# HowToSD/cremage

Hardware: AMD Instinct MI355X
Metric: images/sec SD1.5 512x512 20-step Euler ancestral (txt2img, CFG 7.5, incl. VAE decode) (higher is better)
Workload: dtype bf16; 1 GPU; SD1.5 txt2img 512x512, batch 4 per GPU, 20-step Euler ancestral, bf16 UNet (B=8 with CFG) + fp32-class (split-bf16 x3) VAE decode, synthetic name-keyed weights, synthetic conditioning; sampler=euler_a, sampler_steps=20, parallelism=batch-sharded x1 (weights broadcast 0.00 GB once, images all-gathered per step)

## Files before the change

### cremage_amd/_lib.py

```python
import ctypes as C
import os

_HERE = os.path.dirname(os.path.abspath(__file__))
HALF_F16 = os.environ.get("CRG_HALF", "bf16").lower() in ("f16", "fp16", "float16", "half")
LIB_PATH = os.path.abspath(os.environ["CRG_LIB"]) if os.environ.get("CRG_LIB") else os.path.join(_HERE, "libcrg_hip_f16.so" if HALF_F16 else "libcrg_hip.so")

BF16, F32, F16 = 0, 1, 2
PREC_BF16, PREC_BF16X3, PREC_F16MX = 0, 1, 2
EPI_NONE, EPI_SILU, EPI_GEGLU = 0, 1, 2
BIAS_NONE, BIAS_COL, BIAS_ROW = 0, 1, 2
PACK_LINEAR, PACK_CONV, PACK_GEGLU = 0, 1, 2
K_SLOTS = 17
SLOT_NAMES = ["gemm_w1", "gemm_w4", "gemm_w5", "gemm_x3", "conv_w1", "conv_w4", "conv_w5", "conv_x3", "splitk_reduce", "attention",
              "gn_stats", "gn_apply", "layernorm", "elementwise", "conv_small", "softmax", "lngemm"]
SLOT_FAMILY = ["gemm", "gemm", "gemm", "gemm", "conv", "conv", "conv", "conv", "splitk_reduce", "attention", "groupnorm", "groupnorm",
               "layernorm", "elementwise", "conv_small", "softmax", "gemm"]

c_void_p, c_int, c_int64, c_float, c_size_t = C.c_void_p, C.c_int, C.c_int64, C.c_float, C.c_size_t


class GemmArgs(C.Structure):
    _fields_ = [
        ("a", c_void_p), ("lda", c_int64), ("a_bstride", c_int64),
        ("w", c_void_p), ("ldw", c_int64), ("w_bstride", c_int64),
# ... 80 lines not shown
                              c_int, c_float, c_int, c_int]),
    "crg_groupnorm_split": (c_int, [c_void_p, c_void_p, c_void_p, c_void_p, c_int, c_void_p, c_void_p, c_void_p, c_void_p, c_int, c_int, c_int,
                                    c_int, c_float, c_int]),
    "crg_groupnorm_pre_split": (c_int, [c_void_p, c_void_p, c_void_p, c_void_p, c_void_p, c_void_p, c_void_p, c_void_p, c_int, c_int, c_int, c_int,
                                        c_float, c_int]),
    "crg_groupnorm_pre": (c_int, [c_void_p, c_void_p, c_void_p, c_void_p, c_int, c_void_p, c_void_p, c_void_p, c_void_p, c_void_p, c_int, c_int,
                                  c_int, c_int, c_float, c_int, c_int, c_int, c_int]),
    "crg_split_bf16": (c_int, [c_void_p, c_void_p, c_void_p, c_void_p, c_void_p, c_int64]),
    "crg_split_mx": (c_int, [c_void_p, c_void_p, c_void_p, c_void_p, c_void_p, c_int64, c_int, c_int, c_int]),
    "crg_groupnorm_mx": (c_int, [c_void_p, c_void_p, c_void_p, c_void_p, c_void_p, c_void_p, c_void_p, c_void_p, c_int, c_int, c_int, c_int, c_float,
                                 c_int, c_int, c_int]),
    "crg_pack_weight_mx": (c_int, [c_void_p, c_void_p, c_void_p, c_int, c_int, c_int, c_void_p, c_void_p, c_int, c_int]),
    "crg_layernorm": (c_int, [c_void_p, c_void_p, c_void_p, c_void_p, c_void_p, c_void_p, c_int64, c_int, c_float, c_int]),
    "crg_gemm": (c_int, [c_void_p, c_void_p, C.POINTER(GemmArgs)]),
    "crg_conv2d": (c_int, [c_void_p, c_void_p, C.POINTER(ConvArgs)]),
    "crg_ln_gemm": (c_int, [c_void_p, c_void_p, C.POINTER(LnGemmArgs)]),
    "crg_pack_weight": (c_int, [c_void_p, c_void_p, c_void_p, c_int, c_int, c_int, c_int, c_int, c_void_p, c_void_p]),
    "crg_pack_geglu_bias": (c_int, [c_void_p, c_void_p, c_void_p, c_int, c_void_p]),
    "crg_pack_ln_weight": (c_int, [c_void_p, c_void_p, c_void_p, c_int, c_void_p, c_void_p, c_void_p, c_int, c_int, c_int, c_void_p, c_void_p, c_void_p]),
    "crg_attention": (c_int, [c_void_p, c_void_p, c_void_p, c_int64, c_void_p, c_int64, c_void_p, c_int64, c_void_p, c_int64,
                              c_int, c_int, c_int, c_int, c_int, c_float, c_int]),
    "crg_attention_v": (c_int, [c_void_p, c_void_p, c_void_p, c_int64, c_void_p, c_int64, c_void_p, c_int64, c_void_p, c_int64,
                              c_int, c_int, c_int, c_int, c_int, c_float, c_int]),
    "crg_softmax_rows": (c_int, [c_void_p, c_void_p, c_void_p, c_void_p, c_int64, c_int, c_int64, c_float, c_int]),
    "crg_conv_small": (c_int, [c_void_p, c_void_p, c_void_p, c_void_p, c_void_p, c_void_p, c_int, c_int, c_int, c_int, c_int,
                               c_int, c_int, c_int]),
    "crg_timestep_embedding": (c_int, [c_void_p, c_void_p, c_void_p, c_void_p, c_int, c_int, c_int]),
    "crg_silu": (c_int, [c_void_p, c_void_p, c_void_p, c_void_p, c_int64, c_int]),
    "crg_nchw_to_nhwc": (c_int, [c_void_p, c_void_p, c_void_p, c_void_p, c_int, c_int, c_int, c_int, c_int]),
    "crg_nhwc_to_nchw": (c_int, [c_void_p, c_void_p, c_void_p, c_void_p, c_int, c_int, c_int, c_int, c_int]),
# ... 70 lines not shown
```

### cremage_amd/csrc/crg_api.hip

```cpp
#include "crg_common.h"

int crg_fail(crg_ctx* ctx, int code, const char* fmt, ...) {
  if (ctx) {
    char buf[1024];
    va_list ap;
    va_start(ap, fmt);
    vsnprintf(buf, sizeof(buf), fmt, ap);
    va_end(ap);
    ctx->err = buf;
  }
  return code;
}

void* crg_scratch(crg_ctx* ctx, size_t bytes) {
  if (ctx->scratch_bytes >= bytes) return ctx->scratch;
  size_t want = ctx->scratch_bytes ? ctx->scratch_bytes * 2 : (size_t(64) << 20);
  while (want < bytes) want *= 2;
  void* fresh = nullptr;
  if (hipMalloc(&fresh, want) != hipSuccess) return nullptr;
  if (ctx->scratch) ctx->retired.push_back(ctx->scratch);
  ctx->scratch = fresh;
  ctx->scratch_bytes = want;
  return ctx->scratch;
}
// ... 187 lines not shown
template <typename ST>
__global__ __launch_bounds__(256) void pack_mx_kernel(const ST* __restrict__ src, _Float16* __restrict__ w16, unsigned char* __restrict__ w8,
                                                      int n_in, long total8, float sh, float sl) {
  const int kk = 9 * n_in;
  for (long i = (long)blockIdx.x * 256 + threadIdx.x; i < total8; i += (long)gridDim.x * 256) {
    const long d = i * 8;
    const int o = (int)(d / kk), k = (int)(d - (long)o * kk);
    const int chunk = k / (9 * 64), r = k - chunk * 9 * 64, tap = r / 64, c0 = r - tap * 64;
    float f[8];
#pragma unroll
    for (int e = 0; e < 8; ++e) f[e] = (float)src[((long)o * n_in + chunk * 64 + c0 + e) * 9 + tap];
    crg_store_mx8(f, w16 + d, w8 + 2 * (d - c0) + c0, sh, sl);
  }
}

}

extern "C" int crg_pack_weight_mx(crg_ctx* ctx, void* stream, const void* src, int src_dtype, int n_out, int n_in, void* dst16, void* dst8,
                                  int hi_log2, int lo_log2) {
  if (!ctx) return -22;
  CRG_REQUIRE(ctx, src && dst16 && dst8 && n_out > 0 && n_in > 0 && n_in % 64 == 0, "pack_weight_mx: 3x3 conv weights with Cin %% 64 == 0 (got %d)", n_in);
  const long total8 = (long)n_out * n_in * 9 / 8;
  const int grid = (int)((total8 + 255) / 256 < 4096 ? (total8 + 255) / 256 : 4096);
  hipStream_t st = (hipStream_t)stream;
  const float sh = ldexpf(1.f, hi_log2), sl = ldexpf(1.f, lo_log2);
  if (src_dtype == CRG_F32) hipLaunchKernelGGL(pack_mx_kernel<float>, dim3(grid), dim3(256), 0, st, (const float*)src, (_Float16*)dst16, (unsigned char*)dst8, n_in, total8, sh, sl);
  else if (src_dtype == CRG_BF16) hipLaunchKernelGGL(pack_mx_kernel<bf16>, dim3(grid), dim3(256), 0, st, (const bf16*)src, (_Float16*)dst16, (unsigned char*)dst8, n_in, total8, sh, sl);
  else if (src_dtype == CRG_F16) hipLaunchKernelGGL(pack_mx_kernel<_Float16>, dim3(grid), dim3(256), 0, st, (const _Float16*)src, (_Float16*)dst16, (unsigned char*)dst8, n_in, total8, sh, sl);
  else return crg_fail(ctx, -22, "pack_weight_mx: unsupported source dtype %d", src_dtype);
  CRG_CHECK_LAUNCH(ctx, "pack_weight_mx");
// ... 53 lines not shown
```

### cremage_amd/csrc/gemm_conv.hip

```cpp
#include "gemm_shared.h"
#include <cstdlib>

namespace {
using namespace crg_mm;



__device__ __forceinline__ bf16x8 split_hi(const crg_vec8<float>& v, bf16x8& lo) {
  bf16x8 hi;
#pragma unroll
  for (int i = 0; i < 8; ++i) {
    float f = v.get(i);
    bf16 h = (bf16)f;
    hi[i] = h;
    lo[i] = (bf16)(f - (float)h);
  }
  return hi;
}


template <int WNT, int NSPLIT, typename AT, typename YT, bool CONV, int KG>
__global__ __launch_bounds__(256 * KG) void gemm_kernel(GemmP p) {
  constexpr int BN = 32 * WNT;
  constexpr int RS = 32 * KG;
// ... 622 lines not shown
              V[(long)(n + e) * p.vt_ld] = (bf16)v;
            }
          }
        }
      }
      return;
    }
  }
  if constexpr (PAIR) {
    gemm_epilogue_pairs<WNT, WMT, GST ? 1 : 0, RST>(p, acc, m0, n0, wm, wn, frow, fq, bz, r2, r1, pre_res, bpre, pre_bias);
  } else {
    gemm_epilogue<WNT, YT, WMT>(p, acc, m0, n0, wm, wn, frow, fq, bz, sid, rres, pre_res, bpre, pre_bias);
  }
}

template <int WNT, typename YT, bool PAIR, int NS = 1, int KG = 1, int MT = 1, bool MX = false>
__global__ __launch_bounds__(256 * KG * MT, (KG == 1 && MT == 1) ? 2 : 1) void conv3_rowhalo_kernel(GemmP p) {
  static_assert(!PAIR || (sizeof(YT) == 2 && NS == 1), "paired columns: bf16 output, single-plane operands");
  static_assert(MT == 1 || (KG == 1 && NS == 1), "256-row tiles: single-plane operands, no in-block split-K");
  static_assert(!MX || (NS == 2 && KG == 2 && MT == 1), "MX: the split-plane form on two k-groups");
  constexpr int WMT = 4, NW = 4 * KG * MT;
  constexpr int TP = 128 * MT;
  constexpr int BN = 32 * WNT;
  constexpr int WS_BYTES = BN * 128;
  constexpr int WRG = BN / 8;
  constexpr int WL = (WRG + NW - 1) / NW;
  constexpr int XI = ((MT == 2 ? 36 : 20) + NW - 1) / NW;
  extern __shared__ __attribute__((aligned(16))) char smem[];
  typedef const __attribute__((address_space(1))) void* gptr_t;
  typedef __attribute__((address_space(3))) void* lptr_t;

  const int t = threadIdx.x;
  const int lane = t & 63;
  const int wave = __builtin_amdgcn_readfirstlane(t >> 6);
  const int kg = MT == 2 ? 0 : wave >> 2;
  const int wm = MT == 2 ? wave >> 1 : (wave & 3) >> 1, wn = wave & 1;
  const int Wd = p.Wo, Hd = p.Ho, sh = p.up ? 1 : 0;
  const bool lin = p.halo_lin != 0;
  const bool seg = lin || Wd > TP;
  const int WP = seg ? TP + 2 : Wd + 2;
  const int R = seg ? 1 : TP / Wd;
  const int xpix = R * WP;
  const int XP = (xpix + 7) >> 3;
  const int xbuf_bytes = XP * 1024;
  char* const wring = smem;
  char* const xbuf = smem + 2 * NS * WS_BYTES;

  int tile_m, tile_n, sid;
  block_to_tile(p, tile_m, tile_n, sid);
  const int m0 = tile_m * TP, n0 = tile_n * BN;
  const int bz = 0;
  const bf16* Wp = p.w;
  const long a_lo_off = NS == 2 ? reinterpret_cast<const bf16*>(p.a_lo) - reinterpret_cast<const bf16*>(p.a) : 0;
  const long w_lo_off = NS == 2 ? p.w_lo - p.w : 0;
  const bf16* zpage = p.zero_page;
  const int rsub = lane >> 3;
  const int clog = (lane & 7) ^ rsub;

  int xsrc[XI];
  int xh[XI];
  unsigned xmask[XI];
  {
    const int rows_total = p.M / Wd;
    const int row0 = m0 / Wd;
    const int w0 = m0 - row0 * Wd;
#pragma unroll
    for (int i = 0; i < XI; ++i) {
// ... 20 lines not shown
    }
  }
  bool wok[WL];
  long wrow_off[WL];
#pragma unroll
  for (int q = 0; q < WL; ++q) {
    const int pos = (wave + NW * q) * 8 + rsub;
    const int n = n0 + (PAIR ? unpair_col<WNT>(pos) : pos);
    wok[q] = n < p.N && (wave + NW * q) < WRG;
    wrow_off[q] = (long)n * p.ldw;
  }
  const int g_begin = sid * p.ks_q + (sid < p.ks_r ? sid : p.ks_r);
  const int g_end = g_begin + p.ks_q + (sid < p.ks_r ? 1 : 0);

  auto stage_x = [&](int g, int slot) {
    const int c = g / 3, kh = g - 3 * c;
    const int cch = c * 64 + clog * 8;
    const bool second = cch >= p.C1;
    const bf16* base = reinterpret_cast<const bf16*>(second ? p.x2 : p.a);
    const int Cs = second ? p.C2 : p.C1;
    const int cs = second ? cch - p.C1 : cch;
    char* xb = xbuf + ((g - g_begin) & 1) * (NS * xbuf_bytes);
#pragma unroll
    for (int i = 0; i < XI; ++i) {
      if (i % 3 != slot) continue;
      const int jp = wave + NW * i;
      if (jp < XP) {
        const bool ok = (xmask[i] >> kh) & 1u;
        const bf16* src = ok ? base + (long)(xsrc[i] + ((xh[i] + kh - 1) >> sh) * p.W) * Cs + cs : zpage;
        __builtin_amdgcn_global_load_lds((gptr_t)src, (lptr_t)(xb + jp * 1024), 16, 0, 0);
        if constexpr (NS == 2) {
          const bf16* src2 = ok ? src + a_lo_off : zpage;
          __builtin_amdgcn_global_load_lds((gptr_t)src2, (lptr_t)(xb + xbuf_bytes + jp * 1024), 16, 0, 0);
        }
      }
    }
  };
  auto stage_w = [&](int kt, int buf) {
    char* ws = wring + buf * (NS * WS_BYTES);
    const long kc = (long)kt * BK + clog * 8;
// ... 11 lines not shown
  };

  f32x4 acc[WNT][WMT];
#pragma unroll
  for (int i = 0; i < WNT; ++i)
#pragma unroll
    for (int j = 0; j < WMT; ++j) acc[i][j] = f32x4{0.f, 0.f, 0.f, 0.f};

  const int frow = lane & 15;
  const int fq = lane >> 4;
  int xb0[WMT];
#pragma unroll
  for (int j = 0; j < WMT; ++j) {
    const int ml = wm * 64 + j * 16 + frow;
    const int r = seg ? 0 : ml / Wd;
    xb0[j] = r * WP + (ml - r * Wd);
  }
  unsigned edge = 0;
  if (lin) {
#pragma unroll
    for (int j = 0; j < WMT; ++j) {
      const int m = m0 + wm * 64 + j * 16 + frow;
      const int wcol = m % Wd;
      edge |= (wcol == 0 ? 1u : 0u) << j;
      edge |= (wcol == Wd - 1 ? 1u : 0u) << (8 + j);
    }
  }

  bf16x4 rres[PAIR ? 1 : WNT][PAIR ? 1 : WMT];
  bf16x8 r2[PAIR ? (WNT / 2 > 0 ? WNT / 2 : 1) : 1][PAIR ? WMT : 1];
  bf16x4 r1[PAIR ? WMT : 1];
// ... 25 lines not shown
            rres[i][j] = *reinterpret_cast<const bf16x4*>(Rm + (n + 4 <= p.N ? n : p.N - 4));
          }
        }
      }
    }
    if (pre_bias) {
#pragma unroll
      for (int i = 0; i < WNT; ++i) {
        const int n = (PAIR && i < 2 * (WNT / 2)) ? nb + 32 * (i >> 1) + 8 * fq + 4 * (i & 1) : nb + 16 * i + 4 * fq;
        bpre[i] = *reinterpret_cast<const f32x4*>(p.bias + (n + 4 <= p.N ? n : p.N - 4));
      }
    }
  }

  if (g_begin < g_end) {
    stage_x(g_begin, 0);
    stage_x(g_begin, 1);
    stage_x(g_begin, 2);
    stage_w(3 * g_begin, 0);
  }
#ifdef CRG_X3_NOSTAGGER
  constexpr bool STAG = false;
#else
  constexpr bool STAG = KG == 2 && WNT == 4 && !MX;
#endif
  constexpr bool LO = NS == 2 && !MX;
  bf16x8 sxf[STAG ? WMT : 1], swf[STAG ? WNT : 1], sxl[STAG && LO ? WMT : 1], swl[STAG && LO ? WNT : 1];
  if constexpr (STAG) {
#pragma unroll
    for (int j = 0; j < WMT; ++j) { sxf[j] = bf16x8{0, 0, 0, 0, 0, 0, 0, 0}; if constexpr (LO) sxl[j] = sxf[j]; }
#pragma unroll
    for (int i = 0; i < WNT; ++i) { swf[i] = bf16x8{0, 0, 0, 0, 0, 0, 0, 0}; if constexpr (LO) swl[i] = swf[i]; }
  }
  typedef int v8i __attribute__((ext_vector_type(8)));
// ... 56 lines not shown
            acc[i][j] = CRG_MFMA_16x16x32(swl[i], sxf[j], acc[i][j]);
            acc[i][j] = CRG_MFMA_16x16x32(swf[i], sxl[j], acc[i][j]);
          }
          if constexpr (MX) acc[i][j] = __builtin_amdgcn_mfma_f32_16x16x32_f16(__builtin_bit_cast(h16x8, swf[i]), __builtin_bit_cast(h16x8, sxf[j]), acc[i][j], 0, 0, 0);
          else acc[i][j] = CRG_MFMA_16x16x32(swf[i], sxf[j], acc[i][j]);
        }
      mx_cross();
    }
  };
  int wbuf = 0;
  auto k_loop = [&](auto GBc) {
  constexpr bool GB = decltype(GBc)::value;
  for (int g = g_begin; g < g_end; ++g) {
    const char* xs = xbuf + ((g - g_begin) & 1) * (NS * xbuf_bytes);
#pragma unroll
    for (int kw = 0; kw < 3; ++kw) {
      wait_vmcnt<0>();
      asm volatile("" ::: "memory");
      __builtin_amdgcn_s_barrier();
      asm volatile("" ::: "memory");
      __builtin_amdgcn_s_setprio(2);
      if (kw < 2 || g + 1 < g_end) stage_w(3 * g + kw + 1, wbuf ^ 1);
      if (g + 1 < g_end) stage_x(g + 1, kw);
      __builtin_amdgcn_s_setprio(0);
      const char* ws = wring + wbuf * (NS * WS_BYTES);
      if constexpr (STAG) {
        auto stag_reads = [&]() {
#pragma unroll
          for (int j = 0; j < WMT; ++j) {
            const int off = lds_off(xb0[j] + kw, kg * 4 + fq);
            sxf[j] = *reinterpret_cast<const bf16x8*>(xs + off);
            if constexpr (LO) sxl[j] = *reinterpret_cast<const bf16x8*>(xs + xbuf_bytes + off);
          }
          if (kw != 1 && lin) {
#pragma unroll
            for (int j = 0; j < WMT; ++j) {
              if ((edge >> (kw == 0 ? j : 8 + j)) & 1u) {
// ... 84 lines not shown
#pragma unroll
      for (int i = 0; i < WNT; ++i)
#pragma unroll
        for (int j = 0; j < WMT; ++j) red[(i * WMT + j) * 64] = acc[i][j];
    }
    __syncthreads();
    if (kg == 1) return;
#pragma unroll
    for (int i = 0; i < WNT; ++i)
#pragma unroll
      for (int j = 0; j < WMT; ++j) acc[i][j] += red[(i * WMT + j) * 64];
  }
  if constexpr (PAIR) {
    gemm_epilogue_pairs<WNT, WMT>(p, acc, m0, n0, wm, wn, frow, fq, bz, r2, r1, pre_res, bpre, pre_bias);
  } else {
    gemm_epilogue<WNT, YT, WMT>(p, acc, m0, n0, wm, wn, frow, fq, bz, sid, rres, pre_res, bpre, pre_bias);
  }
}

template <typename YT>
__global__ __launch_bounds__(256) void splitk_reduce_kernel(GemmP p) {
  const int n4 = p.N >> 2;
  const long srows = p.M - p.slab_row0;
  const long total = srows * n4;
  const int bz = blockIdx.y;
  const float* S = p.slab + (long)bz * p.splits * srows * p.N - (long)p.slab_row0 * p.N;
  YT* Y = reinterpret_cast<YT*>(p.y) + (long)bz * p.y_bs;
  const YT* R = p.res ? reinterpret_cast<const YT*>(p.res) + (long)bz * p.r_bs : nullptr;
  for (long idx = (long)blockIdx.x * 256 + threadIdx.x; idx < total; idx += (long)gridDim.x * 256) {
    const int mr = (int)(idx / n4);
    const int m = mr + p.slab_row0;
// ... 552 lines not shown
    p.pair = 0;
    crg_prof_scope ps(ctx, st, CONV ? CRG_K_CONV_X3 : CRG_K_GEMM_X3, wk.flops, wk.bytes);
    hipLaunchKernelGGL(kern, dim3(p.tiles_n * p.tiles_m * p.splits, batch, 1), dim3(512), lds_bytes, st, p);
    CRG_CHECK_LAUNCH(ctx, "gemm(planes)");
  }
  if (p.splits > 1) {
    const long total4 = (long)p.M * (p.N >> 2);
    const int rg = (int)((total4 + 255) / 256 > 2048 ? 2048 : (total4 + 255) / 256);
    crg_prof_scope ps(ctx, st, CRG_K_SPLITK, (double)batch * p.splits * p.M * p.N, (double)batch * p.M * p.N * (4.0 * p.splits + 4));
    hipLaunchKernelGGL(splitk_reduce_kernel<float>, dim3(rg, batch), dim3(256), 0, st, p);
    CRG_CHECK_LAUNCH(ctx, "splitk_reduce");
  }
  return 0;
}

template <int NSPLIT, typename AT, typename YT, bool CONV>
int launch_wnt(crg_ctx* ctx, hipStream_t st, GemmP& p, int batch, Work wk) {
  const bool geglu = p.epi == CRG_EPI_GEGLU;
  if (!geglu && p.N <= 32) return launch<1, NSPLIT, AT, YT, CONV>(ctx, st, p, batch, wk);
  if (!geglu && p.N % 160 == 0) return launch<5, NSPLIT, AT, YT, CONV>(ctx, st, p, batch, wk);
  return launch<4, NSPLIT, AT, YT, CONV>(ctx, st, p, batch, wk);
}

template <bool CONV>
int dispatch(crg_ctx* ctx, hipStream_t st, GemmP& p, int batch, int a_dtype, int y_dtype, int prec, Work wk) {
  const bool gstat_bf16 = prec == CRG_PREC_BF16 && a_dtype == CRG_BF16 && y_dtype == CRG_BF16 && (p.N & 7) == 0;
  const bool gstat_planes = (prec == CRG_PREC_BF16X3 || prec == CRG_PREC_F16MX) && a_dtype == CRG_BF16 && y_dtype == CRG_F32 && p.a_lo && !p.a_is_weight && (p.N & 3) == 0;
  if (p.gstat && !((gstat_bf16 || gstat_planes) && batch == 1 && p.epi == CRG_EPI_NONE))
    return crg_fail(ctx, -22, "gemm/conv: GroupNorm statistics need bf16 in / out (N %% 8 == 0) or pre-split planes in / fp32 out (N %% 4 == 0), batch 1 and a plain epilogue");
  if (prec == CRG_PREC_BF16) {
// ... 142 lines not shown
    CRG_REQUIRE(ctx, (((uintptr_t)a->gn_gamma | (uintptr_t)a->gn_beta | (uintptr_t)a->gn_y) & 15) == 0, "conv2d: GroupNorm pointers must be 16-byte aligned");
    p.gn_gamma = a->gn_gamma; p.gn_beta = a->gn_beta; p.gn_eps = a->gn_eps; p.gn_groups = a->gn_groups; p.gn_silu = a->gn_silu;
    p.gn_hw = a->Ho * a->Wo; p.gn_y = a->gn_y;
  }
  const double flops = 2.0 * p.M * (double)p.N * p.K;
  const double bytes = (double)a->N * a->H * a->W * Ctot * crg_dtype_size(a->x_dtype) + (double)p.N * p.K * 2 +
                       (double)p.M * p.N * crg_dtype_size(a->y_dtype) * (a->residual ? 2 : 1);
  ctx->gn_fused = false;
  const int rc = dispatch<true>(ctx, (hipStream_t)stream, p, 1, a->x_dtype, a->y_dtype, a->prec,
                                Work{flops, bytes, (double)a->N * a->H * a->W * Ctot * crg_dtype_size(a->x_dtype), (double)p.N * p.K * 2});
  if (a->gn_stats_rows) *a->gn_stats_rows = p.gstat_rows;
  if (rc || !a->gn_y || ctx->gn_fused) return rc;
  return crg_groupnorm(ctx, stream, a->y, nullptr, a->Cout, a->gn_gamma, a->gn_beta, a->gn_y, a->N, a->Ho * a->Wo, a->Cout, a->gn_groups,
                       a->gn_eps, a->gn_silu, a->y_dtype);
}
```

### cremage_amd/csrc/gemm_shared.h

```cpp
#pragma once
#include "crg_common.h"
#include <type_traits>

namespace crg_mm {

struct GemmP {
  const void* a; const void* a_lo; long lda, a_bs;
  const bf16* w; const bf16* w_lo; long ldw, w_bs;
  const float* bias; int bias_mode;
  const void* res; long ldr, r_bs;
  void* y; long ldy, y_bs;
  int M, N, K, epi;
  const float* cvec; int cvec_rows; long cvec_ld;
  const bf16* zero_page;
  int splits; float* slab;
  int a_is_weight;
  const void* x2; int C1, C2, Ctot, H, W, Ho, Wo, ks, stride, pad_t, pad_l, up;
  int cm;
  int tiles_n, tiles_m;
  int tile_base, tile_count, slab_row0;
  int pair;
  int rowhalo;
  int halo_lin;
  int ks_q, ks_r;
// ... 37 lines not shown
  }
}

__device__ __forceinline__ int lds_off(int row, int chunk) { return row * 128 + ((chunk ^ (row & 7)) << 4); }

__device__ __forceinline__ float row16_sum(float v) {
#if defined(__HIP_DEVICE_COMPILE__)
  v += __builtin_bit_cast(float, __builtin_amdgcn_update_dpp(0, __builtin_bit_cast(int, v), 0xB1, 0xF, 0xF, true));
  v += __builtin_bit_cast(float, __builtin_amdgcn_update_dpp(0, __builtin_bit_cast(int, v), 0x4E, 0xF, 0xF, true));
  v += __builtin_bit_cast(float, __builtin_amdgcn_update_dpp(0, __builtin_bit_cast(int, v), 0x141, 0xF, 0xF, true));
  v += __builtin_bit_cast(float, __builtin_amdgcn_update_dpp(0, __builtin_bit_cast(int, v), 0x140, 0xF, 0xF, true));
#endif
  return v;
}

template <int WNT, typename YT, int WMT = 4>
__device__ __forceinline__ void gemm_epilogue(const GemmP& p, f32x4 (&acc)[WNT][WMT], int m0, int n0, int wm, int wn, int frow, int fq,
                                              int bz, int sid, const bf16x4 (&pre)[WNT][WMT], bool use_pre,
                                              const f32x4 (&bpre)[WNT], bool use_bpre) {
  if (p.splits > 1) {
    const long srows = p.M - p.slab_row0;
    float* S = p.slab + ((long)bz * p.splits + sid) * srows * p.N - (long)p.slab_row0 * p.N;
#pragma unroll
    for (int j = 0; j < WMT; ++j) {
      const int m = m0 + wm * (16 * WMT) + j * 16 + frow;
      if (m >= p.M) continue;
#pragma unroll
      for (int i = 0; i < WNT; ++i) {
        const int n = n0 + wn * (16 * WNT) + i * 16 + fq * 4;
        if (n + 4 <= p.N) {
          *reinterpret_cast<f32x4*>(S + (long)m * p.N + n) = acc[i][j];
        } else {
          for (int e = 0; e < 4 && n + e < p.N; ++e) S[(long)m * p.N + n + e] = acc[i][j][e];
        }
      }
    }
    return;
  }
  YT* Y = reinterpret_cast<YT*>(p.y) + (long)bz * p.y_bs;
  const YT* R = p.res ? reinterpret_cast<const YT*>(p.res) + (long)bz * p.r_bs : nullptr;
  constexpr bool CAN_STATS = sizeof(YT) == 4 && (WMT % 2 == 0);
  const bool do_stats = CAN_STATS && p.gstat != nullptr;
  f32x4 gs1[CAN_STATS ? WNT : 1], gs2[CAN_STATS ? WNT : 1];
  auto flush_stats = [&](int jb) {
    if constexpr (CAN_STATS) {
      const int row0 = m0 + wm * (16 * WMT) + jb * 16;
      const long rb = row0 >> 5;
#pragma unroll
      for (int i = 0; i < WNT; ++i) {
        f32x4 a, b;
#pragma unroll
        for (int e = 0; e < 4; ++e) {
          a[e] = row16_sum(gs1[i][e]);
          b[e] = row16_sum(gs2[i][e]);
        }
        const int n = n0 + wn * (16 * WNT) + i * 16 + fq * 4;
        if (frow == 0 && n + 4 <= p.N && row0 < p.M) {
          *reinterpret_cast<f32x4*>(p.gstat + rb * p.N + n) = a;
          *reinterpret_cast<f32x4*>(p.gstat + p.gstat_plane + rb * p.N + n) = b;
        }
      }
    }
  };
#pragma unroll
  for (int j = 0; j < WMT; ++j) {
    const int m = m0 + wm * (16 * WMT) + j * 16 + frow;
    if constexpr (CAN_STATS) {
      if (do_stats && (j & 1) == 0) {
        if (j > 0) flush_stats(j - 2);
#pragma unroll
        for (int i = 0; i < WNT; ++i) gs1[i] = gs2[i] = f32x4{0.f, 0.f, 0.f, 0.f};
      }
    }
    if (m >= p.M) continue;
    const float brow = (p.bias_mode == CRG_BIAS_ROW) ? p.bias[m] : 0.f;
    const float* cv = p.cvec ? p.cvec + (long)(m / p.cvec_rows) * p.cvec_ld : nullptr;
    if (p.epi == CRG_EPI_GEGLU) {
      if constexpr (WNT % 2 == 0) {
#pragma unroll
        for (int u = 0; u < WNT / 2; ++u) {
          const int pn = n0 + wn * (16 * WNT) + u * 32 + fq * 4;
          if (pn >= p.N) continue;
          const int jn = (n0 + wn * (16 * WNT)) / 2 + u * 16 + fq * 4;
          f32x4 v = acc[2 * u][j], g = acc[2 * u + 1][j];
          if (p.bias_mode == CRG_BIAS_COL) {
            v += *reinterpret_cast<const f32x4*>(p.bias + pn);
            g += *reinterpret_cast<const f32x4*>(p.bias + pn + 16);
          }
          YT out[4];
// ... 9 lines not shown
#pragma unroll
    for (int i = 0; i < WNT; ++i) {
      const int n = n0 + wn * (16 * WNT) + i * 16 + fq * 4;
      if (n >= p.N) continue;
      f32x4 v = acc[i][j];
      const bool full = (n + 4 <= p.N);
      if (full) {
        if (use_bpre) v += bpre[i];
        else if (p.bias_mode == CRG_BIAS_COL) v += *reinterpret_cast<const f32x4*>(p.bias + n);
        else if (p.bias_mode == CRG_BIAS_ROW) v += brow;
        if (p.epi == CRG_EPI_SILU) {
#pragma unroll
          for (int e = 0; e < 4; ++e) v[e] = crg_silu_f(v[e]);
        }
        if (cv) v += *reinterpret_cast<const f32x4*>(cv + n);
        const long yo = (long)m * p.ldy + n;
        if (use_pre) {
#pragma unroll
          for (int e = 0; e < 4; ++e) v[e] += (float)pre[i][j][e];
        } else if (R) {
          const YT* rp = R + (long)m * p.ldr + n;
          if (((p.ldr | n) & 3) == 0) {
            if constexpr (sizeof(YT) == 2) {
              bf16x4 r4 = *reinterpret_cast<const bf16x4*>(rp);
#pragma unroll
              for (int e = 0; e < 4; ++e) v[e] += (float)r4[e];
            } else {
              v += *reinterpret_cast<const f32x4*>(rp);
            }
          } else {
#pragma unroll
// ... 15 lines not shown
          } else {
            *reinterpret_cast<f32x4*>(Y + yo) = v;
          }
        } else {
#pragma unroll
          for (int e = 0; e < 4; ++e) Y[yo + e] = (YT)v[e];
        }
      } else {
        for (int e = 0; e < 4 && n + e < p.N; ++e) {
          float s = v[e];
          if (p.bias_mode == CRG_BIAS_COL) s += p.bias[n + e];
          else if (p.bias_mode == CRG_BIAS_ROW) s += brow;
          if (p.epi == CRG_EPI_SILU) s = crg_silu_f(s);
          if (cv) s += cv[n + e];
          if (R) s += (float)R[(long)m * p.ldr + n + e];
          Y[(long)m * p.ldy + n + e] = (YT)s;
        }
      }
    }
  }
  if constexpr (CAN_STATS) {
    if (do_stats) flush_stats(WMT - 2);
  }
}

template <int WNT>
__device__ __forceinline__ int unpair_col(int pos) {
  const int w = pos / (16 * WNT);
  const int l = pos - w * (16 * WNT);
  if (l >= 32 * (WNT / 2)) return pos;
  const int g = l >> 5, t = (l >> 4) & 1, rho = l & 15;
// ... 239 lines not shown
```

### cremage_amd/ops.py

```python
from __future__ import annotations

import ctypes as C
from typing import Optional, Tuple

import torch

from . import _lib as L

HALF = torch.float16 if L.HALF_F16 else torch.bfloat16
_DT = {HALF: L.BF16, torch.float32: L.F32}
if not L.HALF_F16:
    _DT[torch.float16] = L.F16


def _dt(t: torch.Tensor) -> int:
    try:
        return _DT[t.dtype]
    except KeyError:
        raise L.CrgError(f"unsupported dtype {t.dtype}")


def _act_dt(t: torch.Tensor) -> int:
    if t.dtype not in (HALF, torch.float32):
        raise L.CrgError(f"activations must be {HALF} or float32, got {t.dtype}")
# ... 191 lines not shown
    src = w.detach().contiguous()
    if src.dtype not in _DT:
        src = src.float()
    n_out = src.shape[0]
    if kind == L.PACK_CONV:
        n_in, ks = src.shape[1], src.shape[2]
        cols = n_in * ks * ks
    else:
        n_in, ks = src[0].numel(), 1
        cols = n_in
    hi = torch.empty((n_out, cols), dtype=HALF, device=w.device)
    lo = torch.empty_like(hi) if split else None
    h = _h(w)
    L.check(L.load().crg_pack_weight(h, _st(), _p(src), _dt(src), kind, n_out, n_in, ks, _p(hi), _p(lo)), h, "crg_pack_weight")
    return _pack_cache.put((w,), (kind, split), (hi, lo))


VAE_MX = __import__("os").environ.get("CRG_VAE_MX", "0") != "0"
MX_X_LOG2 = (4, 15)


def packed_weight_mx(w: torch.Tensor):
    _need_cuda(w)
    r = _pack_cache.get((w,), ("mx",))
    if r is not None:
        return r
    src = w.detach().contiguous()
    if src.dtype not in _DT:
        src = src.float()
    n_out, n_in = src.shape[0], src.shape[1]
# ... 437 lines not shown
    ho = (hv + pt + pb - ks) // stride + 1
    wo = (wv + pl + pr - ks) // stride + 1
    if cin <= 8 or (cin == 9 and cout % 8 == 0) or (cout <= 8 and (cin % 8 != 0 or cin < 64)):
        if x_lo is not None:
            raise L.CrgError("conv2d: thin-channel convs take the fp32 tensor, not split planes")
        if stride != 1 or upsample2x or x2 is not None or cvec is not None or residual is not None or gn is not None or (pt, pl, pb, pr) != (ks // 2,) * 4:
            raise L.CrgError("conv2d: thin-channel convs support only stride 1, 'same' padding, no fusions (no fused GroupNorm either)")
        y = empty_image(n, cout, ho, wo, x.dtype, x.device)
        w32 = f32_vec(weight)
        h = _h(x)
        L.check(L.load().crg_conv_small(h, _st(), _p(x), _p(w32), _p(f32_vec(bias)), _p(y), n, hh, ww, cin, cout, ks, _act_dt(x),
                                        _act_dt(y)), h, "crg_conv_small")
        return y
    planes = x_lo is not None
    split = planes or x.dtype == torch.float32
    hi, lo = packed_weight(weight, L.PACK_CONV, split)
    y = empty_image(n, cout, ho, wo, torch.float32 if planes else x.dtype, x.device)
    if residual is not None:
        residual = to_channels_last(residual)
        if residual.shape != y.shape or residual.dtype != y.dtype:
            raise L.CrgError("conv2d: residual must match the output in shape and dtype")
    if cvec is not None:
        if cvec.dtype != torch.float32 or tuple(cvec.shape) != (n, cout) or cvec.stride(1) != 1 or cvec.stride(0) % 4:
            raise L.CrgError("conv2d: cvec must be fp32 [N, Cout] with unit column stride and 16-byte aligned rows")
    a = L.ConvArgs(x=x.data_ptr(), x2=x2.data_ptr() if x2 is not None else None, C1=c1, C2=c2, w=hi.data_ptr(),
                   w_lo=lo.data_ptr() if lo is not None else None, bias=_p(f32_vec(bias)).value, cvec=_p(cvec).value,
                   cvec_ld=cvec.stride(0) if cvec is not None else 0, residual=_p(residual).value, y=y.data_ptr(), N=n, H=hh, W=ww, Cout=cout, Ho=ho, Wo=wo, ksize=ks, stride=stride,
                   pad_t=pt, pad_l=pl, upsample2x=int(upsample2x), x_dtype=_act_dt(x), y_dtype=_act_dt(y),
                   prec=L.PREC_BF16X3 if planes else _prec(x), x_lo=x_lo.data_ptr() if planes else None)
    y_norm = keep = None
    if gn is not None:
# ... 1 lines not shown
        if planes or y.dtype != HALF or cout % groups or (cout // groups) % 8:
            raise L.CrgError("conv2d: the fused GroupNorm takes bf16 outputs with 8-aligned groups")
        y_norm = empty_image(n, cout, ho, wo, y.dtype, x.device)
        keep = (f32_vec(gw), f32_vec(gb))
        a.gn_gamma, a.gn_beta, a.gn_y = keep[0].data_ptr(), keep[1].data_ptr(), y_norm.data_ptr()
        a.gn_groups, a.gn_silu, a.gn_eps = int(groups), int(bool(silu)), float(eps)
    stats = _gn_stats_buffer(n * ho * wo, cout, ho * wo, x.dtype, y.dtype, x.device) if (gn_stats and gn is None and (planes or x.dtype == HALF)) else None
    if stats is not None and planes and (cout % 4 or VAE_GN_STATS is False):
        stats = None
    rows = C.c_int(32)
    if stats is not None:
        a.gn_stats = stats.data_ptr()
        if GN_TILE and not planes:
            a.gn_stats_rows = C.pointer(rows)
    h = _h(x)
    L.check(L.load().crg_conv2d(h, _st(), C.byref(a)), h, "crg_conv2d")
    if stats is not None:
        y._crg_gn = (stats, y._version, ho * wo, rows.value)
    return y if gn is None else (y, y_norm)


def _conv2d_mx(x16, x8, weight, bias, stride, padding, upsample2x, x2, cvec, residual, x_lo, gn_stats, gn):
    x16 = to_channels_last(x16)
    n, c, hh, ww = x16.shape
    cout, cin, ks, _ = weight.shape
    if x16.dtype != torch.float16 or x8.dtype != torch.uint8 or tuple(x8.shape) != (n, hh, ww, 2 * c) or not x8.is_contiguous():
        raise L.CrgError("conv2d(x_mx=): x must be the fp16 plane [N, C, H, W] (channels-last) and x_mx the uint8 plane [N, H, W, 2 C]")
    if ks != 3 or stride != 1 or padding not in (1, (1, 1, 1, 1)) or upsample2x or x2 is not None or x_lo is not None or gn is not None or cvec is not None \
            or cin != c or c % 64:
        raise L.CrgError("conv2d(x_mx=): 3x3 / stride 1 / pad 1 convs with Cin % 64 == 0 only (no upsample / concat / fused GroupNorm)")
    w16, w8, whi, wlo = packed_weight_mx(weight)
# ... 251 lines not shown
```

### include/crg_hip.h

```cpp
#ifndef CRG_HIP_H
#define CRG_HIP_H

#include <stddef.h>
#include <stdint.h>

#ifdef __cplusplus
extern "C" {
#endif

#define CRG_VERSION 103

typedef struct crg_ctx crg_ctx;

enum crg_dtype { CRG_BF16 = 0, CRG_F32 = 1, CRG_F16 = 2 };

enum crg_prec { CRG_PREC_BF16 = 0, CRG_PREC_BF16X3 = 1,
                CRG_PREC_F16MX = 2 };

enum crg_epilogue {
  CRG_EPI_NONE = 0,
  CRG_EPI_SILU = 1,
  CRG_EPI_GEGLU = 2
};

// ... 86 lines not shown
  int64_t cvec_ld;
  const void* residual;
  void* y;
  int N, H, W, Cout, Ho, Wo;
  int ksize, stride, pad_t, pad_l;
  int upsample2x;
  int x_dtype, y_dtype, prec;
  const void* x_lo;
  float* gn_stats;
  const float* gn_gamma; const float* gn_beta; void* gn_y;
  int gn_groups; int gn_silu; float gn_eps;
  int mx_log2[4];
  int* gn_stats_rows;
} crg_conv_args;
int crg_conv2d(crg_ctx* ctx, void* stream, const crg_conv_args* args);

enum crg_pack_kind { CRG_PACK_LINEAR = 0, CRG_PACK_CONV = 1, CRG_PACK_GEGLU = 2 };
int crg_pack_weight(crg_ctx* ctx, void* stream, const void* src, int src_dtype, int kind, int n_out, int n_in,
                    int ksize, void* dst_hi, void* dst_lo);
int crg_pack_geglu_bias(crg_ctx* ctx, void* stream, const float* src, int n_out2, float* dst);
int crg_pack_ln_weight(crg_ctx* ctx, void* stream, const void* src, int src_dtype, const float* gamma, const float* beta,
                       const float* bias, int kind, int n_out, int n_in, void* dst_w, float* dst_colsum, float* dst_bias);

int crg_attention(crg_ctx* ctx, void* stream, const void* q, int64_t ldq, const void* k, int64_t ldk,
                  const void* vt, int64_t ldvt, void* o, int64_t ldo, int B, int H, int Nq, int Nk, int Dh,
                  float scale, int dtype);
int crg_attention_v(crg_ctx* ctx, void* stream, const void* q, int64_t ldq, const void* k, int64_t ldk,
                    const void* v, int64_t ldv, void* o, int64_t ldo, int B, int H, int Nq, int Nk, int Dh,
                    float scale, int dtype);

int crg_softmax_rows(crg_ctx* ctx, void* stream, const void* x, void* y, int64_t rows, int cols, int64_t ld,
                     float scale, int dtype);

int crg_conv_small(crg_ctx* ctx, void* stream, const void* x, const float* w, const float* bias, void* y,
// ... 52 lines not shown
```

Baseline: 17.87 images/s.

## Fold nearest-2x upsample into VAE 3x3 conv via sub-pixel 2x2 weight classes

Replaces the nearest-upsample-then-3x3-conv in the VAE decoder with four 2x2 convolutions on the low-resolution input, one per output sub-pixel phase. The weights are pre-summed per phase into a packed hi/lo bf16 layout, and the epilogue scatters rows to interleaved output positions and to matching GroupNorm stat blocks. This cuts conv K from 9*Cin to 4*Cin per output pixel and avoids reading an upsampled image. The cost is a new kernel specialisation and a pre-summed weight pack whose rounding differs slightly from the plain path.

```diff
diff --git a/cremage_amd/_lib.py b/cremage_amd/_lib.py
--- a/cremage_amd/_lib.py
+++ b/cremage_amd/_lib.py
@@ -118,6 +118,8 @@
     "crg_layernorm": (c_int, [c_void_p, c_void_p, c_void_p, c_void_p, c_void_p, c_void_p, c_int64, c_int, c_float, c_int]),
     "crg_gemm": (c_int, [c_void_p, c_void_p, C.POINTER(GemmArgs)]),
     "crg_conv2d": (c_int, [c_void_p, c_void_p, C.POINTER(ConvArgs)]),
+    "crg_conv2d_subpix": (c_int, [c_void_p, c_void_p, C.POINTER(ConvArgs)]),
+    "crg_pack_weight_subpix": (c_int, [c_void_p, c_void_p, c_void_p, c_int, c_int, c_int, c_void_p, c_void_p]),
     "crg_ln_gemm": (c_int, [c_void_p, c_void_p, C.POINTER(LnGemmArgs)]),
     "crg_pack_weight": (c_int, [c_void_p, c_void_p, c_void_p, c_int, c_int, c_int, c_int, c_int, c_void_p, c_void_p]),
     "crg_pack_geglu_bias": (c_int, [c_void_p, c_void_p, c_void_p, c_int, c_void_p]),
diff --git a/cremage_amd/csrc/crg_api.hip b/cremage_amd/csrc/crg_api.hip
--- a/cremage_amd/csrc/crg_api.hip
+++ b/cremage_amd/csrc/crg_api.hip
@@ -225,6 +225,42 @@
   }
 }
 
+template <typename ST>
+__global__ __launch_bounds__(256) void pack_subpix_kernel(const ST* __restrict__ src, bf16* __restrict__ hi, bf16* __restrict__ lo, int n_out,
+                                                          int n_in, long total) {
+  for (long d = (long)blockIdx.x * 256 + threadIdx.x; d < total; d += (long)gridDim.x * 256) {
+    const long kk = 4L * n_in;
+    const long co = d / kk;
+    const int k = (int)(d - co * kk);
+    const int cls = (int)(co / n_out), o = (int)(co - (long)cls * n_out);
+    const int chunk = k >> 8, tap = (k >> 6) & 3, ci = chunk * 64 + (k & 63);
+    const int a = cls >> 1, b = cls & 1, r = tap >> 1, t = tap & 1;
+    const int h0 = a == 0 ? (r == 0 ? 0 : 1) : (r == 0 ? 0 : 2), h1 = a == 0 ? (r == 0 ? 0 : 2) : (r == 0 ? 1 : 2);
+    const int w0 = b == 0 ? (t == 0 ? 0 : 1) : (t == 0 ? 0 : 2), w1 = b == 0 ? (t == 0 ? 0 : 2) : (t == 0 ? 1 : 2);
+    const ST* s = src + ((long)o * n_in + ci) * 9;
+    float f = 0.f;
+    for (int kh = h0; kh <= h1; ++kh)
+      for (int kw = w0; kw <= w1; ++kw) f += (float)s[kh * 3 + kw];
+    const bf16 h = (bf16)f;
+    hi[d] = h;
+    lo[d] = (bf16)(f - (float)h);
+  }
+}
+
+}
+
+extern "C" int crg_pack_weight_subpix(crg_ctx* ctx, void* stream, const void* src, int src_dtype, int n_out, int n_in, void* dst_hi, void* dst_lo) {
+  if (!ctx) return -22;
+  CRG_REQUIRE(ctx, src && dst_hi && dst_lo && n_out > 0 && n_in > 0 && n_in % 64 == 0, "pack_weight_subpix: 3x3 conv weights with Cin %% 64 == 0 (got %d)", n_in);
+  const long total = 16L * n_out * n_in;
+  const int grid = (int)((total + 255) / 256 < 4096 ? (total + 255) / 256 : 4096);
+  hipStream_t st = (hipStream_t)stream;
+  if (src_dtype == CRG_F32) hipLaunchKernelGGL(pack_subpix_kernel<float>, dim3(grid), dim3(256), 0, st, (const float*)src, (bf16*)dst_hi, (bf16*)dst_lo, n_out, n_in, total);
+  else if (src_dtype == CRG_BF16) hipLaunchKernelGGL(pack_subpix_kernel<bf16>, dim3(grid), dim3(256), 0, st, (const bf16*)src, (bf16*)dst_hi, (bf16*)dst_lo, n_out, n_in, total);
+  else if (src_dtype == CRG_F16) hipLaunchKernelGGL(pack_subpix_kernel<_Float16>, dim3(grid), dim3(256), 0, st, (const _Float16*)src, (bf16*)dst_hi, (bf16*)dst_lo, n_out, n_in, total);
+  else return crg_fail(ctx, -22, "pack_weight_subpix: unsupported source dtype %d", src_dtype);
+  CRG_CHECK_LAUNCH(ctx, "pack_weight_subpix");
+  return 0;
 }
 
 extern "C" int crg_pack_weight_mx(crg_ctx* ctx, void* stream, const void* src, int src_dtype, int n_out, int n_in, void* dst16, void* dst8,
diff --git a/cremage_amd/csrc/gemm_conv.hip b/cremage_amd/csrc/gemm_conv.hip
--- a/cremage_amd/csrc/gemm_conv.hip
+++ b/cremage_amd/csrc/gemm_conv.hip
@@ -660,11 +660,13 @@
   }
 }
 
-template <int WNT, typename YT, bool PAIR, int NS = 1, int KG = 1, int MT = 1, bool MX = false>
+template <int WNT, typename YT, bool PAIR, int NS = 1, int KG = 1, int MT = 1, bool MX = false, bool SUB = false>
 __global__ __launch_bounds__(256 * KG * MT, (KG == 1 && MT == 1) ? 2 : 1) void conv3_rowhalo_kernel(GemmP p) {
   static_assert(!PAIR || (sizeof(YT) == 2 && NS == 1), "paired columns: bf16 output, single-plane operands");
   static_assert(MT == 1 || (KG == 1 && NS == 1), "256-row tiles: single-plane operands, no in-block split-K");
   static_assert(!MX || (NS == 2 && KG == 2 && MT == 1), "MX: the split-plane form on two k-groups");
+  static_assert(!SUB || (NS == 2 && KG == 2 && MT == 1 && !MX && !PAIR), "sub-pixel upsample: the bf16 x 3 split-plane form");
+  constexpr int KW = SUB ? 2 : 3;
   constexpr int WMT = 4, NW = 4 * KG * MT;
   constexpr int TP = 128 * MT;
   constexpr int BN = 32 * WNT;
@@ -681,8 +683,8 @@
   const int wave = __builtin_amdgcn_readfirstlane(t >> 6);
   const int kg = MT == 2 ? 0 : wave >> 2;
   const int wm = MT == 2 ? wave >> 1 : (wave & 3) >> 1, wn = wave & 1;
-  const int Wd = p.Wo, Hd = p.Ho, sh = p.up ? 1 : 0;
-  const bool lin = p.halo_lin != 0;
+  const int Wd = SUB ? p.W : p.Wo, Hd = SUB ? p.H : p.Ho, sh = (p.up && !SUB) ? 1 : 0;
+  const bool lin = !SUB && p.halo_lin != 0;
   const bool seg = lin || Wd > TP;
   const int WP = seg ? TP + 2 : Wd + 2;
   const int R = seg ? 1 : TP / Wd;
@@ -694,9 +696,15 @@
 
   int tile_m, tile_n, sid;
   block_to_tile(p, tile_m, tile_n, sid);
+  int cls = 0;
+  if constexpr (SUB) {
+    cls = tile_m & 3;
+    tile_m >>= 2;
+  }
+  const int pa = cls >> 1, pb = cls & 1;
   const int m0 = tile_m * TP, n0 = tile_n * BN;
   const int bz = 0;
-  const bf16* Wp = p.w;
+  const bf16* Wp = p.w + (SUB ? (long)cls * p.N * p.ldw : 0);
   const long a_lo_off = NS == 2 ? reinterpret_cast<const bf16*>(p.a_lo) - reinterpret_cast<const bf16*>(p.a) : 0;
   const long w_lo_off = NS == 2 ? p.w_lo - p.w : 0;
   const bf16* zpage = p.zero_page;
@@ -747,7 +755,7 @@
   const int g_end = g_begin + p.ks_q + (sid < p.ks_r ? 1 : 0);
 
   auto stage_x = [&](int g, int slot) {
-    const int c = g / 3, kh = g - 3 * c;
+    const int c = g / KW, kh = (g - KW * c) + (SUB ? pa : 0);
     const int cch = c * 64 + clog * 8;
     const bool second = cch >= p.C1;
     const bf16* base = reinterpret_cast<const bf16*>(second ? p.x2 : p.a);
@@ -756,7 +764,7 @@
     char* xb = xbuf + ((g - g_begin) & 1) * (NS * xbuf_bytes);
 #pragma unroll
     for (int i = 0; i < XI; ++i) {
-      if (i % 3 != slot) continue;
+      if (i % KW != slot) continue;
       const int jp = wave + NW * i;
       if (jp < XP) {
         const bool ok = (xmask[i] >> kh) & 1u;
@@ -798,7 +806,7 @@
   for (int j = 0; j < WMT; ++j) {
     const int ml = wm * 64 + j * 16 + frow;
     const int r = seg ? 0 : ml / Wd;
-    xb0[j] = r * WP + (ml - r * Wd);
+    xb0[j] = r * WP + (ml - r * Wd) + (SUB ? pb : 0);
   }
   unsigned edge = 0;
   if (lin) {
@@ -854,10 +862,9 @@
   }
 
   if (g_begin < g_end) {
-    stage_x(g_begin, 0);
-    stage_x(g_begin, 1);
-    stage_x(g_begin, 2);
-    stage_w(3 * g_begin, 0);
+#pragma unroll
+    for (int slot = 0; slot < KW; ++slot) stage_x(g_begin, slot);
+    stage_w(KW * g_begin, 0);
   }
 #ifdef CRG_X3_NOSTAGGER
   constexpr bool STAG = false;
@@ -944,13 +951,13 @@
   for (int g = g_begin; g < g_end; ++g) {
     const char* xs = xbuf + ((g - g_begin) & 1) * (NS * xbuf_bytes);
 #pragma unroll
-    for (int kw = 0; kw < 3; ++kw) {
+    for (int kw = 0; kw < KW; ++kw) {
       wait_vmcnt<0>();
       asm volatile("" ::: "memory");
       __builtin_amdgcn_s_barrier();
       asm volatile("" ::: "memory");
       __builtin_amdgcn_s_setprio(2);
-      if (kw < 2 || g + 1 < g_end) stage_w(3 * g + kw + 1, wbuf ^ 1);
+      if (kw < KW - 1 || g + 1 < g_end) stage_w(KW * g + kw + 1, wbuf ^ 1);
       if (g + 1 < g_end) stage_x(g + 1, kw);
       __builtin_amdgcn_s_setprio(0);
       const char* ws = wring + wbuf * (NS * WS_BYTES);
@@ -1065,7 +1072,7 @@
   if constexpr (PAIR) {
     gemm_epilogue_pairs<WNT, WMT>(p, acc, m0, n0, wm, wn, frow, fq, bz, r2, r1, pre_res, bpre, pre_bias);
   } else {
-    gemm_epilogue<WNT, YT, WMT>(p, acc, m0, n0, wm, wn, frow, fq, bz, sid, rres, pre_res, bpre, pre_bias);
+    gemm_epilogue<WNT, YT, WMT, SUB>(p, acc, m0, n0, wm, wn, frow, fq, bz, sid, rres, pre_res, bpre, pre_bias, cls);
   }
 }
 
@@ -1648,6 +1655,30 @@
   return 0;
 }
 
+int launch_planes_sub(crg_ctx* ctx, hipStream_t st, GemmP& p, Work wk) {
+  constexpr int WNT = 4, BN = 32 * WNT;
+  p.zero_page = (const bf16*)ctx->zero_page;
+  p.tiles_n = (p.N + BN - 1) / BN;
+  p.tiles_m = 4 * ((p.M + 127) / 128);
+  p.splits = 1;
+  p.slab = nullptr;
+  choose_xcd_partition(p, wk);
+  p.tile_base = 0;
+  p.tile_count = p.tiles_n * p.tiles_m;
+  p.slab_row0 = 0;
+  p.ks_q = (p.K / BK) / 2;
+  p.ks_r = 0;
+  p.pair = 0;
+  void (*kern)(GemmP) = conv3_rowhalo_kernel<WNT, float, false, 2, 2, 1, false, true>;
+  const int XP = p.W > 128 ? 17 : ((128 / p.W) * (p.W + 2) + 7) / 8;
+  const size_t lds_bytes = (size_t)2 * 2 * BN * 128 + (size_t)2 * 2 * XP * 1024;
+  if (int rc = crg_set_dyn_lds(ctx, reinterpret_cast<const void*>(kern), (size_t)2 * 2 * BN * 128 + 2 * 2 * 18 * 1024, "conv2d_subpix")) return rc;
+  crg_prof_scope ps(ctx, st, CRG_K_CONV_X3, wk.flops, wk.bytes);
+  hipLaunchKernelGGL(kern, dim3(p.tiles_n * p.tiles_m), dim3(512), lds_bytes, st, p);
+  CRG_CHECK_LAUNCH(ctx, "conv2d_subpix");
+  return 0;
+}
+
 template <int NSPLIT, typename AT, typename YT, bool CONV>
 int launch_wnt(crg_ctx* ctx, hipStream_t st, GemmP& p, int batch, Work wk) {
   const bool geglu = p.epi == CRG_EPI_GEGLU;
@@ -1820,3 +1851,39 @@
   return crg_groupnorm(ctx, stream, a->y, nullptr, a->Cout, a->gn_gamma, a->gn_beta, a->gn_y, a->N, a->Ho * a->Wo, a->Cout, a->gn_groups,
                        a->gn_eps, a->gn_silu, a->y_dtype);
 }
+
+extern "C" int crg_conv2d_subpix(crg_ctx* ctx, void* stream, const crg_conv_args* a) {
+  if (!ctx || !a) return -22;
+  CRG_REQUIRE(ctx, a->N > 0 && a->H > 0 && a->W > 0 && a->Cout > 0, "conv2d_subpix: empty problem");
+  CRG_REQUIRE(ctx, a->ksize == 3 && a->stride == 1 && a->pad_t == 1 && a->pad_l == 1 && a->upsample2x && a->Ho == 2 * a->H && a->Wo == 2 * a->W,
+              "conv2d_subpix: a nearest-2x upsample followed by a 3x3 / stride 1 / pad 1 conv (output %dx%d from %dx%d)", a->Ho, a->Wo, a->H, a->W);
+  CRG_REQUIRE(ctx, a->prec == CRG_PREC_BF16X3 && a->x_dtype == CRG_BF16 && a->y_dtype == CRG_F32 && a->x_lo && a->w_lo && !a->x2 && a->C2 == 0,
+              "conv2d_subpix: pre-split bf16 planes (x / x_lo, w / w_lo) in, fp32 out, BF16X3, no second input");
+  CRG_REQUIRE(ctx, a->C1 % 64 == 0 && a->Cout > 32 && a->Cout % 160 != 0 && a->Cout % 4 == 0,
+              "conv2d_subpix: Cin %% 64 == 0 and a 128-wide output tile (Cout > 32, Cout %% 160 != 0, Cout %% 4 == 0); got Cin %d Cout %d", a->C1, a->Cout);
+  CRG_REQUIRE(ctx, a->W >= 16 && (a->W <= 128 ? 128 % a->W == 0 : a->W % 128 == 0) && (a->H * a->W) % 32 == 0,
+              "conv2d_subpix: source width %d must divide 128 (>= 16) or be a multiple of it, H * W a multiple of 32", a->W);
+  CRG_REQUIRE(ctx, !a->residual && !a->cvec && !a->gn_y, "conv2d_subpix: no residual, channel vector or fused GroupNorm");
+  CRG_REQUIRE(ctx, ((uintptr_t)a->x & 15) == 0 && ((uintptr_t)a->x_lo & 15) == 0 && ((uintptr_t)a->w & 15) == 0 && ((uintptr_t)a->w_lo & 15) == 0 &&
+                       ((uintptr_t)a->bias & 15) == 0 && ((uintptr_t)a->y & 15) == 0 && ((uintptr_t)a->gn_stats & 15) == 0,
+              "conv2d_subpix: pointers must be 16-byte aligned");
+  CRG_REQUIRE(ctx, (double)a->N * a->Ho * a->Wo < 2147483648.0, "conv2d_subpix: problem too large");
+  GemmP p{};
+  p.a = a->x; p.a_lo = a->x_lo; p.x2 = nullptr; p.C1 = a->C1; p.C2 = 0; p.Ctot = a->C1;
+  p.w = (const bf16*)a->w; p.w_lo = (const bf16*)a->w_lo; p.ldw = 4L * a->C1; p.w_bs = 0;
+  p.bias = a->bias; p.bias_mode = a->bias ? CRG_BIAS_COL : CRG_BIAS_NONE;
+  p.res = nullptr; p.ldr = a->Cout; p.r_bs = 0;
+  p.y = a->y; p.ldy = a->Cout; p.y_bs = 0;
+  p.M = a->N * a->H * a->W; p.N = a->Cout; p.K = 4 * a->C1; p.epi = CRG_EPI_NONE;
+  p.cvec = nullptr; p.cvec_rows = 1; p.cvec_ld = 0;
+  p.H = a->H; p.W = a->W; p.Ho = a->Ho; p.Wo = a->Wo; p.ks = 3; p.stride = 1; p.pad_t = 1; p.pad_l = 1; p.up = 1;
+  p.cm = 1; p.rowhalo = 1; p.halo_lin = 0;
+  const long mo = (long)a->N * a->Ho * a->Wo;
+  p.gstat = a->gn_stats; p.gstat_plane = (mo / 32) * p.N;
+  p.gstat_rows = 32;
+  const double flops = 2.0 * mo * p.N * p.K;
+  const double xb = (double)p.M * p.C1 * 2.0 * 2, wb = 4.0 * p.N * p.K * 2 * 2;
+  const int rc = launch_planes_sub(ctx, (hipStream_t)stream, p, Work{flops, xb + wb + (double)mo * p.N * 4, xb, wb});
+  if (a->gn_stats_rows) *a->gn_stats_rows = 32;
+  return rc;
+}
diff --git a/cremage_amd/csrc/gemm_shared.h b/cremage_amd/csrc/gemm_shared.h
--- a/cremage_amd/csrc/gemm_shared.h
+++ b/cremage_amd/csrc/gemm_shared.h
@@ -75,10 +75,17 @@
   return v;
 }
 
-template <int WNT, typename YT, int WMT = 4>
+__device__ __forceinline__ long sub_out_row(const GemmP& p, int m, int cls) {
+  const int hw = p.H * p.W;
+  const int img = m / hw, r = m - img * hw, y = r / p.W, x = r - y * p.W;
+  return ((long)img * (2 * p.H) + 2 * y + (cls >> 1)) * (2 * p.W) + 2 * x + (cls & 1);
+}
+
+template <int WNT, typename YT, int WMT = 4, bool SUB = false>
 __device__ __forceinline__ void gemm_epilogue(const GemmP& p, f32x4 (&acc)[WNT][WMT], int m0, int n0, int wm, int wn, int frow, int fq,
                                               int bz, int sid, const bf16x4 (&pre)[WNT][WMT], bool use_pre,
-                                              const f32x4 (&bpre)[WNT], bool use_bpre) {
+                                              const f32x4 (&bpre)[WNT], bool use_bpre, int cls = 0) {
+  static_assert(!SUB || sizeof(YT) == 4, "sub-pixel rows: the fp32-class epilogue only");
   if (p.splits > 1) {
     const long srows = p.M - p.slab_row0;
     float* S = p.slab + ((long)bz * p.splits + sid) * srows * p.N - (long)p.slab_row0 * p.N;
@@ -106,7 +113,11 @@
   auto flush_stats = [&](int jb) {
     if constexpr (CAN_STATS) {
       const int row0 = m0 + wm * (16 * WMT) + jb * 16;
-      const long rb = row0 >> 5;
+      long rb = row0 >> 5;
+      if constexpr (SUB) {
+        const int hw = p.H * p.W, img = row0 / hw;
+        rb = ((long)img * 4 + cls) * (hw >> 5) + ((row0 - img * hw) >> 5);
+      }
 #pragma unroll
       for (int i = 0; i < WNT; ++i) {
         f32x4 a, b;
@@ -134,6 +145,7 @@
       }
     }
     if (m >= p.M) continue;
+    const long ym = SUB ? sub_out_row(p, m, cls) : (long)m;
     const float brow = (p.bias_mode == CRG_BIAS_ROW) ? p.bias[m] : 0.f;
     const float* cv = p.cvec ? p.cvec + (long)(m / p.cvec_rows) * p.cvec_ld : nullptr;
     if (p.epi == CRG_EPI_GEGLU) {
@@ -173,7 +185,7 @@
           for (int e = 0; e < 4; ++e) v[e] = crg_silu_f(v[e]);
         }
         if (cv) v += *reinterpret_cast<const f32x4*>(cv + n);
-        const long yo = (long)m * p.ldy + n;
+        const long yo = ym * p.ldy + n;
         if (use_pre) {
 #pragma unroll
           for (int e = 0; e < 4; ++e) v[e] += (float)pre[i][j][e];
@@ -219,7 +231,7 @@
           if (p.epi == CRG_EPI_SILU) s = crg_silu_f(s);
           if (cv) s += cv[n + e];
           if (R) s += (float)R[(long)m * p.ldr + n + e];
-          Y[(long)m * p.ldy + n + e] = (YT)s;
+          Y[ym * p.ldy + n + e] = (YT)s;
         }
       }
     }
diff --git a/cremage_amd/ops.py b/cremage_amd/ops.py
--- a/cremage_amd/ops.py
+++ b/cremage_amd/ops.py
@@ -229,6 +229,43 @@
     h = _h(w)
     L.check(L.load().crg_pack_weight(h, _st(), _p(src), _dt(src), kind, n_out, n_in, ks, _p(hi), _p(lo)), h, "crg_pack_weight")
     return _pack_cache.put((w,), (kind, split), (hi, lo))
+
+
+VAE_SUBPIX = __import__("os").environ.get("CRG_VAE_SUBPIX", "1") != "0"
+SUBPIX_ROWS = (((0,), (1, 2)), ((0, 1), (2,)))
+
+
+def subpixel_weights(w: torch.Tensor) -> torch.Tensor:
+    cls = []
+    for a in (0, 1):
+        for b in (0, 1):
+            t = torch.stack([torch.stack([sum(w[:, :, kh, kw] for kh in SUBPIX_ROWS[a][r] for kw in SUBPIX_ROWS[b][c]) for c in (0, 1)], -1)
+                             for r in (0, 1)], -2)
+            cls.append(t)
+    return torch.stack(cls, 0)
+
+
+def packed_weight_subpix(w: torch.Tensor) -> Tuple[torch.Tensor, torch.Tensor]:
+    _need_cuda(w)
+    r = _pack_cache.get((w,), ("subpix",))
+    if r is not None:
+        return r
+    src = w.detach().contiguous()
+    if src.dtype not in _DT:
+        src = src.float()
+    n_out, n_in = src.shape[0], src.shape[1]
+    hi = torch.empty((4 * n_out, 4 * n_in), dtype=HALF, device=w.device)
+    lo = torch.empty_like(hi)
+    h = _h(w)
+    L.check(L.load().crg_pack_weight_subpix(h, _st(), _p(src), _dt(src), n_out, n_in, _p(hi), _p(lo)), h, "crg_pack_weight_subpix")
+    return _pack_cache.put((w,), ("subpix",), (hi, lo))
+
+
+def subpix_ok(x: torch.Tensor, weight: torch.Tensor) -> bool:
+    n, c, hh, ww = x.shape
+    cout, cin, ks, ks2 = weight.shape
+    return (VAE_SUBPIX and ks == 3 and ks2 == 3 and cin == c and cin % 64 == 0 and cout > 32 and cout % 160 != 0 and cout % 4 == 0 and
+            ww >= 16 and (128 % ww == 0 if ww <= 128 else ww % 128 == 0) and (hh * ww) % 32 == 0 and n * 4 * hh * ww < 2 ** 31)
 
 
 VAE_MX = __import__("os").environ.get("CRG_VAE_MX", "0") != "0"
@@ -696,7 +733,9 @@
         return y
     planes = x_lo is not None
     split = planes or x.dtype == torch.float32
-    hi, lo = packed_weight(weight, L.PACK_CONV, split)
+    subpix = (planes and upsample2x and stride == 1 and (pt, pl, pb, pr) == (1, 1, 1, 1) and x2 is None and cvec is None and residual is None and
+              gn is None and subpix_ok(x, weight))
+    hi, lo = packed_weight_subpix(weight) if subpix else packed_weight(weight, L.PACK_CONV, split)
     y = empty_image(n, cout, ho, wo, torch.float32 if planes else x.dtype, x.device)
     if residual is not None:
         residual = to_channels_last(residual)
@@ -728,7 +767,10 @@
         if GN_TILE and not planes:
             a.gn_stats_rows = C.pointer(rows)
     h = _h(x)
-    L.check(L.load().crg_conv2d(h, _st(), C.byref(a)), h, "crg_conv2d")
+    if subpix:
+        L.check(L.load().crg_conv2d_subpix(h, _st(), C.byref(a)), h, "crg_conv2d_subpix")
+    else:
+        L.check(L.load().crg_conv2d(h, _st(), C.byref(a)), h, "crg_conv2d")
     if stats is not None:
         y._crg_gn = (stats, y._version, ho * wo, rows.value)
     return y if gn is None else (y, y_norm)
diff --git a/include/crg_hip.h b/include/crg_hip.h
--- a/include/crg_hip.h
+++ b/include/crg_hip.h
@@ -124,10 +124,12 @@
   int* gn_stats_rows;
 } crg_conv_args;
 int crg_conv2d(crg_ctx* ctx, void* stream, const crg_conv_args* args);
+int crg_conv2d_subpix(crg_ctx* ctx, void* stream, const crg_conv_args* args);
 
 enum crg_pack_kind { CRG_PACK_LINEAR = 0, CRG_PACK_CONV = 1, CRG_PACK_GEGLU = 2 };
 int crg_pack_weight(crg_ctx* ctx, void* stream, const void* src, int src_dtype, int kind, int n_out, int n_in,
                     int ksize, void* dst_hi, void* dst_lo);
+int crg_pack_weight_subpix(crg_ctx* ctx, void* stream, const void* src, int src_dtype, int n_out, int n_in, void* dst_hi, void* dst_lo);
 int crg_pack_geglu_bias(crg_ctx* ctx, void* stream, const float* src, int n_out2, float* dst);
 int crg_pack_ln_weight(crg_ctx* ctx, void* stream, const void* src, int src_dtype, const float* gamma, const float* beta,
                        const float* bias, int kind, int n_out, int n_in, void* dst_w, float* dst_colsum, float* dst_bias);
```

Measured after the change: 18.12 images/s (median of 6 runs). +1.4%, better.
